# ewrfcas/MVSFormer

Hardware: AMD Instinct MI355X
Metric: depth maps/sec @1536x1152 N=5 D=192 (higher is better)
Workload: dtype f32

## Files before the change

### mvsformer_amd/csrc/vis_net_x3.hip

```cpp
#include <stdlib.h>

#include <type_traits>

#include "conv_common.h"
#include "split3.h"

#ifdef X3_ABLATE
#define VIS_ABLATE(a, bit) (((a) & (bit)) != 0)
static int vis_ablate_bits() { return mvs::env_int("MVS_VIS_ABLATE", 0); }
#else
#define VIS_ABLATE(a, bit) false
static constexpr int vis_ablate_bits() { return 0; }
#endif

namespace {
using namespace mvsconv;
using mvsx3::bf16x4;
using mvsx3::bf16x8;
using mvsx3::mfma6;
using mvsprim::u32x2;
using mvsx3::split3;

constexpr int T = 16;
constexpr int INW = T + 6, A1W = T + 4, A2W = T + 2;
constexpr int A1N = A1W * A1W, A2N = A2W * A2W;
constexpr int A1_OCT = A1N * 16, A1_TERM = 2 * A1_OCT;
constexpr int A2_OCT = A2N * 16, A2_TERM = 2 * A2_OCT;
constexpr int IN_BYTES = ((INW * INW * 4 + 255) / 256) * 256;
constexpr int IDX_BYTES = A1N * 4;
constexpr int LDS_BYTES = IN_BYTES + 3 * A1_TERM + 3 * A2_TERM + IDX_BYTES;
constexpr int L2_STEPS = 5, L3_STEPS = 6;
constexpr int L2_FLAT = A2W * A1W;
constexpr int L2_TILES = (L2_FLAT + 15) / 16, L1_TILES = A1N / 16;
static_assert(A1N % 16 == 0, "layer 1 tiles are full");
constexpr int OFF_W0 = 0, OFF_S0 = 144, OFF_B0 = 160, OFF_W1 = 176, OFF_S1 = 2480, OFF_B1 = 2496, OFF_W2 = 2512, OFF_S2 = 3664,
              OFF_B2 = 3672, OFF_W3 = 3680, OFF_B3 = 3688;

__global__ void vis_x3_prepare_kernel(const float* __restrict__ prm, bf16x8* __restrict__ out) {
    const int idx = blockIdx.x * blockDim.x + threadIdx.x;
    if (idx >= (L2_STEPS + L3_STEPS) * 3 * 64) return;
    const int lane = idx & 63, term = (idx >> 6) % 3, step = idx / 192;
    const int m = lane & 15, kb = lane >> 4;
    bf16x8 v;
#pragma unroll
    for (int e = 0; e < 8; ++e) {
        const int ci = (kb & 1) * 8 + e;
        float f = 0.0f;
        if (step < L2_STEPS) {
            const int tap = 2 * step + (kb >> 1);
            if (tap < 9) f = prm[OFF_W1 + (ci * 9 + tap) * 16 + m] * prm[OFF_S1 + m];
        } else {
            const int kblk = 2 * (step - L2_STEPS) + (kb >> 1), t = kblk / 3, kw = kblk % 3, dy = m >> 3, co = m & 7, kh = t - dy;
            if (kh >= 0 && kh <= 2) f = prm[OFF_W2 + (ci * 9 + kh * 3 + kw) * 8 + co] * prm[OFF_S2 + co];
        }
        __bf16 h, mm, l;
        split3(f, h, mm, l);
        v[e] = term == 0 ? h : (term == 1 ? mm : l);
    }
    out[idx] = v;
}

template <int OCT, int TERM>
__device__ __forceinline__ void store_split(unsigned char* base, int pix, int kb, const float (&v)[4]) {
    u32x2 h, m, l;
#pragma unroll
    for (int r = 0; r < 2; ++r) {
        unsigned a, b, c;
#ifdef VIS_SPLIT_CLAMPED
        mvsx3::split3_pair<true>(v[2 * r], v[2 * r + 1], a, b, c);
#else
        mvsx3::split3_pair<false>(v[2 * r], v[2 * r + 1], a, b, c);
#endif
        h[r] = a; m[r] = b; l[r] = c;
    }
    unsigned char* dst = base + (kb >> 1) * OCT + pix * 16 + (kb & 1) * 8;
    *reinterpret_cast<u32x2*>(dst) = h;
    *reinterpret_cast<u32x2*>(dst + TERM) = m;
    *reinterpret_cast<u32x2*>(dst + 2 * TERM) = l;
}

__global__ __launch_bounds__(256, 2) void vis_x3_kernel(const float* __restrict__ entropy, const float* __restrict__ prm,
                                                        const bf16x8* __restrict__ prep, int N, int H, int W, int ntx, int nty,
                                                        float* __restrict__ weight, int ablate) {
    extern __shared__ __attribute__((aligned(16))) unsigned char smem[];
    float* s_in = reinterpret_cast<float*>(smem);
    unsigned char* s_a1 = smem + IN_BYTES;
    unsigned char* s_a2 = s_a1 + 3 * A1_TERM;
    unsigned* s_idx = reinterpret_cast<unsigned*>(s_a2 + 3 * A2_TERM);
    const int tid = threadIdx.x, lane = tid & 63;
    const int wave = __builtin_amdgcn_readfirstlane(tid >> 6);
    const int n = lane & 15, kb = lane >> 4;

    bf16x8 w2[L2_STEPS][3], w3[L3_STEPS][3];
#pragma unroll
    for (int s = 0; s < L2_STEPS; ++s)
#pragma unroll
        for (int t = 0; t < 3; ++t) w2[s][t] = prep[(s * 3 + t) * 64 + lane];
#pragma unroll
    for (int s = 0; s < L3_STEPS; ++s)
#pragma unroll
        for (int t = 0; t < 3; ++t) w3[s][t] = prep[((L2_STEPS + s) * 3 + t) * 64 + lane];

    float W1A[3];
    int tap_off[3];
#pragma unroll
    for (int t = 0; t < 3; ++t) {
        const int tap = 4 * t + kb;
        W1A[t] = tap < 9 ? prm[OFF_W0 + tap * 16 + n] * prm[OFF_S0 + n] : 0.0f;
        const int tc = tap < 9 ? tap : 8;
        tap_off[t] = (tc / 3) * INW + tc % 3;
    }
    f32x4 sh0, sh1, sh2;
    float wl[4];
#pragma unroll
    for (int r = 0; r < 4; ++r) {
        sh0[r] = prm[OFF_B0 + 4 * kb + r];
        sh1[r] = prm[OFF_B1 + 4 * kb + r];
        const int co = (kb & 1) * 4 + r;
        sh2[r] = prm[OFF_B2 + co];
        wl[r] = prm[OFF_W3 + co];
    }
    const float b3 = prm[OFF_B3];
    unsigned off2[L2_STEPS], off3[L3_STEPS];
#pragma unroll
    for (int s = 0; s < L2_STEPS; ++s) {
        const int tap = min(2 * s + (kb >> 1), 8);
        off2[s] = (unsigned)((kb & 1) * A1_OCT + ((tap / 3) * A1W + tap % 3) * 16);
    }
#pragma unroll
    for (int s = 0; s < L3_STEPS; ++s) {
        const int kblk = 2 * s + (kb >> 1);
        off3[s] = (unsigned)((kb & 1) * A2_OCT + ((kblk / 3) * A2W + kblk % 3) * 16);
    }

    const int ntiles = N * ntx * nty;
    constexpr int EPT = (INW * INW + 255) / 256;
    float pre[EPT];
    auto tile_origin = [&](int tile, int& img, int& x0, int& y0) {
        img = tile / (ntx * nty);
        y0 = ((tile / ntx) % nty) * T;
        x0 = (tile % ntx) * T;
    };
    auto fetch_entropy = [&](int tile) {
        int img, x0, y0;
        tile_origin(tile, img, x0, y0);
        const float* src = entropy + (size_t)img * H * W;
#pragma unroll
        for (int e = 0; e < EPT; ++e) {
            const int i = tid + e * 256;
            const int gy = y0 - 3 + i / INW, gx = x0 - 3 + i % INW;
            pre[e] = (i < INW * INW && gy >= 0 && gy < H && gx >= 0 && gx < W) ? src[(size_t)gy * W + gx] : 0.0f;
        }
    };
    auto commit_entropy = [&]() {
#pragma unroll
        for (int e = 0; e < EPT; ++e)
            if (tid + e * 256 < INW * INW) s_in[tid + e * 256] = pre[e];
    };

    int tile = blockIdx.x;
    if (tile >= ntiles) return;
    fetch_entropy(tile);
    commit_entropy();
    for (int p = tid; p < A1N; p += 256) {
        const int py = p / A1W, px = p % A1W;
        s_idx[p] = (unsigned)((py * INW + px) * 4) | (unsigned)py << 16 | (unsigned)px << 24;
    }
    __syncthreads();
    for (; tile < ntiles; tile += gridDim.x) {
        int img, x0, y0;
        tile_origin(tile, img, x0, y0);
        const int next = tile + gridDim.x;
        const bool has_next = next < ntiles;
        if (has_next) fetch_entropy(next);

        const bool interior = x0 >= 2 && y0 >= 2 && x0 + T + 2 <= W && y0 + T + 2 <= H;

        auto layer1 = [&](auto inner) {
            constexpr bool INNER = decltype(inner)::value;
#pragma unroll 1
            for (int t = wave; t < L1_TILES && !VIS_ABLATE(ablate, 1); t += 4) {
                const int p = t * 16 + n;
                const unsigned ix = s_idx[p];
                const float* src = reinterpret_cast<const float*>(reinterpret_cast<const unsigned char*>(s_in) + (ix & 0xffffu));
                f32x4 z = sh0;
#pragma unroll
                for (int k = 0; k < 3; ++k) z = mfma4(W1A[k], src[tap_off[k]], z);
                float cap = __builtin_inff();
                if (!INNER) {
                    const int gy = y0 - 2 + (int)((ix >> 16) & 0xffu), gx = x0 - 2 + (int)(ix >> 24);
                    cap = (gy >= 0 && gy < H && gx >= 0 && gx < W) ? __builtin_inff() : 0.0f;
                }
                float v[4];
#pragma unroll
                for (int r = 0; r < 4; ++r) v[r] = INNER ? fmaxf(z[r], 0.0f) : __builtin_amdgcn_fmed3f(z[r], 0.0f, cap);
                store_split<A1_OCT, A1_TERM>(s_a1, p, kb, v);
            }
        };
        if (interior) layer1(std::true_type{}); else layer1(std::false_type{});
        __syncthreads();

#pragma unroll 1
        for (int t = wave; t < L2_TILES; t += 8) {
            const int o0 = t * 16 + n, o1 = min(t + 4, L2_TILES - 1) * 16 + n;
            const bool two = t + 4 < L2_TILES;
            const unsigned char* b0 = s_a1 + o0 * 16;
            const unsigned char* b1 = s_a1 + o1 * 16;
            f32x4 c0 = sh1, c1 = sh1;
            bf16x8 x0f[2][3], x1f[2][3];
#pragma unroll
            for (int k = 0; k < 3; ++k) {
                x0f[0][k] = *reinterpret_cast<const bf16x8*>(b0 + off2[0] + k * A1_TERM);
                x1f[0][k] = *reinterpret_cast<const bf16x8*>(b1 + off2[0] + k * A1_TERM);
            }
#ifndef VIS_SETPRIO
#define VIS_SETPRIO 1
#endif
            if (VIS_SETPRIO) __builtin_amdgcn_s_setprio(1);
#pragma unroll
            for (int s = 0; s < L2_STEPS; ++s) {
                if (s + 1 < L2_STEPS) {
#pragma unroll
                    for (int k = 0; k < 3; ++k) {
                        x0f[(s + 1) & 1][k] = *reinterpret_cast<const bf16x8*>(b0 + off2[s + 1] + k * A1_TERM);
                        x1f[(s + 1) & 1][k] = *reinterpret_cast<const bf16x8*>(b1 + off2[s + 1] + k * A1_TERM);
                    }
                }
                __builtin_amdgcn_sched_barrier(0);
                if (!VIS_ABLATE(ablate, 2)) {
                    c0 = mfma6(w2[s], x0f[s & 1], c0);
                    c1 = mfma6(w2[s], x1f[s & 1], c1);
                }
                __builtin_amdgcn_sched_barrier(0);
            }
            if (VIS_SETPRIO) __builtin_amdgcn_s_setprio(0);
            auto finish = [&](int tt, const f32x4& c) {
                const int o = tt * 16 + n, oy = o / A1W, ox = o % A1W;
                if (oy < A2W && ox < A2W) {
                    float v[4];
                    if (interior) {
#pragma unroll
                        for (int r = 0; r < 4; ++r) v[r] = fmaxf(c[r], 0.0f);
                    } else {
                        const int gy = y0 - 1 + oy, gx = x0 - 1 + ox;
                        const float cap = (gy >= 0 && gy < H && gx >= 0 && gx < W) ? __builtin_inff() : 0.0f;
#pragma unroll
                        for (int r = 0; r < 4; ++r) v[r] = __builtin_amdgcn_fmed3f(c[r], 0.0f, cap);
                    }
                    store_split<A2_OCT, A2_TERM>(s_a2, oy * A2W + ox, kb, v);
                }
            };
            if (!VIS_ABLATE(ablate, 4)) {
                finish(t, c0);
                if (two) finish(t + 4, c1);
            }
        }
        if (has_next) commit_entropy();
        __syncthreads();

        {
            const unsigned char* b0 = s_a2 + ((2 * wave) * A2W + n) * 16;
            const unsigned char* b1 = s_a2 + ((2 * (wave + 4)) * A2W + n) * 16;
            f32x4 c0 = sh2, c1 = sh2;
            bf16x8 x0f[2][3], x1f[2][3];
#pragma unroll
            for (int k = 0; k < 3; ++k) {
                x0f[0][k] = *reinterpret_cast<const bf16x8*>(b0 + off3[0] + k * A2_TERM);
                x1f[0][k] = *reinterpret_cast<const bf16x8*>(b1 + off3[0] + k * A2_TERM);
            }
            if (VIS_SETPRIO) __builtin_amdgcn_s_setprio(1);
#pragma unroll
            for (int s = 0; s < L3_STEPS; ++s) {
                if (s + 1 < L3_STEPS) {
#pragma unroll
                    for (int k = 0; k < 3; ++k) {
                        x0f[(s + 1) & 1][k] = *reinterpret_cast<const bf16x8*>(b0 + off3[s + 1] + k * A2_TERM);
                        x1f[(s + 1) & 1][k] = *reinterpret_cast<const bf16x8*>(b1 + off3[s + 1] + k * A2_TERM);
                    }
                }
                __builtin_amdgcn_sched_barrier(0);
                if (!VIS_ABLATE(ablate, 8)) {
                    c0 = mfma6(w3[s], x0f[s & 1], c0);
                    c1 = mfma6(w3[s], x1f[s & 1], c1);
                }
                __builtin_amdgcn_sched_barrier(0);
            }
            if (VIS_SETPRIO) __builtin_amdgcn_s_setprio(0);
            auto reduce = [&](const f32x4& c) {
                float part = 0.0f;
#pragma unroll
                for (int r = 0; r < 4; ++r) part = fmaf(wl[r], fmaxf(c[r], 0.0f), part);
                return part + __shfl_xor(part, 16, 64);
            };
            if (!VIS_ABLATE(ablate, 16)) {
                const float p0 = reduce(c0), p1 = reduce(c1);
                const bool second = (kb & 1) != 0;
                const float part = second ? p1 : p0;
                const int gy = y0 + 2 * (second ? wave + 4 : wave) + (kb >> 1), gx = x0 + n;
                if (gy < H && gx < W) weight[(size_t)img * H * W + (size_t)gy * W + gx] = 1.0f / (1.0f + expf(-(part + b3)));
            }
        }
    }
}

}

extern "C" int mvs_vis_x3_prepare(const float* params, void* prepared, mvs_stream_t stream) {
    MVS_REQUIRE(params && prepared, "mvs_vis_x3_prepare: null pointer");
    constexpr int total = (L2_STEPS + L3_STEPS) * 3 * 64;
    static_assert(total * 16 == MVS_VIS_X3_BYTES, "MVS_VIS_X3_BYTES");
    hipLaunchKernelGGL(vis_x3_prepare_kernel, dim3(mvs::ceil_div(total, 256)), dim3(256), 0, MVS_STREAM(stream), params, static_cast<bf16x8*>(prepared));
    return mvs::finish_launch("mvs_vis_x3_prepare");
}

extern "C" int mvs_vis_x3_fwd(const float* entropy, const float* params, const void* prepared, int N, int H, int W, float* weight,
                              mvs_stream_t stream) {
    MVS_REQUIRE(entropy && params && prepared && weight, "mvs_vis_x3_fwd: null pointer");
    MVS_REQUIRE(N >= 1 && H >= 1 && W >= 1, "mvs_vis_x3_fwd: bad shape N=%d H=%d W=%d", N, H, W);
    const int ntx = mvs::ceil_div(W, T), nty = mvs::ceil_div(H, T);
    MVS_REQUIRE((int64_t)N * ntx * nty < ((int64_t)1 << 31), "mvs_vis_x3_fwd: too many tiles");
    const int ncu = mvs::device_cus();
    const int ntiles = N * ntx * nty;
    const int blocks = ntiles < 2 * ncu ? ntiles : 2 * ncu;
    {
        const int rc = mvs::ensure_dynamic_lds(reinterpret_cast<const void*>(&vis_x3_kernel), LDS_BYTES, "mvs_vis_x3_fwd");
        if (rc != MVS_OK) return rc;
    }
    hipLaunchKernelGGL(vis_x3_kernel, dim3(blocks), dim3(256), LDS_BYTES, MVS_STREAM(stream), entropy, params, static_cast<const bf16x8*>(prepared), N,
                       H, W, ntx, nty, weight, vis_ablate_bits());
    return mvs::finish_launch("mvs_vis_x3_fwd");
}
```

Measured before the change: 269.1.

## Software-pipeline layer-2 epilogue into next tile's MFMA stream

Restructures the layer-2 conv loop so each wave processes one tile per pass and interleaves the previous tile's ReLU, bf16x3 split and LDS stores, one piece after each MFMA. A trash pixel slot is added to A2 so out-of-range outputs store unconditionally instead of branching. The goal is to hide epilogue VALU and LDS-store latency behind matrix instructions. In exchange the code is more complex, uses more registers, and loses the two-tile accumulator pairing, so MFMA dependency chains get longer.

```diff
diff --git a/mvsformer_amd/csrc/vis_net_x3.hip b/mvsformer_amd/csrc/vis_net_x3.hip
--- a/mvsformer_amd/csrc/vis_net_x3.hip
+++ b/mvsformer_amd/csrc/vis_net_x3.hip
@@ -1,6 +1,7 @@
 #include <stdlib.h>
 
 #include <type_traits>
+#include <utility>
 
 #include "conv_common.h"
 #include "split3.h"
@@ -25,7 +26,8 @@
 constexpr int INW = T + 6, A1W = T + 4, A2W = T + 2;
 constexpr int A1N = A1W * A1W, A2N = A2W * A2W;
 constexpr int A1_OCT = A1N * 16, A1_TERM = 2 * A1_OCT;
-constexpr int A2_OCT = A2N * 16, A2_TERM = 2 * A2_OCT;
+constexpr int A2_TRASH = A2N;
+constexpr int A2_OCT = (A2N + 1) * 16, A2_TERM = 2 * A2_OCT;
 constexpr int IN_BYTES = ((INW * INW * 4 + 255) / 256) * 256;
 constexpr int IDX_BYTES = A1N * 4;
 constexpr int LDS_BYTES = IN_BYTES + 3 * A1_TERM + 3 * A2_TERM + IDX_BYTES;
@@ -79,6 +81,67 @@
     *reinterpret_cast<u32x2*>(dst + 2 * TERM) = l;
 }
 
+struct L2Epi {
+    f32x4 c;
+    int o, oy, pix;
+    unsigned dst;
+    float cap;
+    f32x4 v;
+    mvsprim::f32x2 ra, rb;
+    u32x2 h, m, l;
+};
+constexpr int L2_EPI_STEPS = 22;
+static_assert(L2_EPI_STEPS <= 6 * L2_STEPS, "one piece behind each MFMA of a pass");
+template <int J, bool INNER>
+__device__ __forceinline__ void l2_epi_step(L2Epi& e, unsigned char* s_a2, unsigned st_lane, int x0, int y0, int H, int W) {
+    if constexpr (J == 0) {
+        e.oy = e.o / A1W;
+    } else if constexpr (J == 1) {
+        const int ox = e.o - e.oy * A1W;
+        e.pix = (e.oy < A2W && ox < A2W) ? e.oy * A2W + ox : A2_TRASH;
+        if (!INNER) {
+            const int gy = y0 - 1 + e.oy, gx = x0 - 1 + ox;
+            e.cap = (gy >= 0 && gy < H && gx >= 0 && gx < W) ? __builtin_inff() : 0.0f;
+        }
+    } else if constexpr (J == 2) {
+        e.dst = st_lane + (unsigned)e.pix * 16u;
+    } else if constexpr (J == 3 || J == 4) {
+#pragma unroll
+        for (int r = 2 * (J - 3); r < 2 * (J - 3) + 2; ++r) e.v[r] = INNER ? fmaxf(e.c[r], 0.0f) : __builtin_amdgcn_fmed3f(e.c[r], 0.0f, e.cap);
+    } else if constexpr (J >= 5 && J < 19) {
+        constexpr int r = (J - 5) & 1, P = (J - 5) >> 1;
+        if constexpr (P == 0) {
+#ifdef VIS_SPLIT_CLAMPED
+            e.h[r] = mvsx3::cvt_pk_bf16(__builtin_amdgcn_fmed3f(e.v[2 * r], -mvsx3::BF16_MAX, mvsx3::BF16_MAX),
+                                        __builtin_amdgcn_fmed3f(e.v[2 * r + 1], -mvsx3::BF16_MAX, mvsx3::BF16_MAX));
+#else
+            e.h[r] = mvsx3::cvt_pk_bf16(e.v[2 * r], e.v[2 * r + 1]);
+#endif
+        } else if constexpr (P == 1) {
+            e.ra[r] = e.v[2 * r] - __builtin_bit_cast(float, e.h[r] << 16);
+        } else if constexpr (P == 2) {
+            e.rb[r] = e.v[2 * r + 1] - __builtin_bit_cast(float, e.h[r] & 0xffff0000u);
+        } else if constexpr (P == 3) {
+            e.m[r] = mvsx3::cvt_pk_bf16(e.ra[r], e.rb[r]);
+        } else if constexpr (P == 4) {
+            e.ra[r] = e.ra[r] - __builtin_bit_cast(float, e.m[r] << 16);
+        } else if constexpr (P == 5) {
+            e.rb[r] = e.rb[r] - __builtin_bit_cast(float, e.m[r] & 0xffff0000u);
+        } else {
+            e.l[r] = mvsx3::cvt_pk_bf16(e.ra[r], e.rb[r]);
+        }
+    } else if constexpr (J == 19) {
+        *reinterpret_cast<u32x2*>(s_a2 + e.dst) = e.h;
+    } else if constexpr (J == 20) {
+        *reinterpret_cast<u32x2*>(s_a2 + e.dst + A2_TERM) = e.m;
+    } else if constexpr (J == 21) {
+        *reinterpret_cast<u32x2*>(s_a2 + e.dst + 2 * A2_TERM) = e.l;
+    }
+}
+template <class F, int... I>
+__device__ __forceinline__ void for_each_int(F&& f, std::integer_sequence<int, I...>) {
+    (f(std::integral_constant<int, I>{}), ...);
+}
 __global__ __launch_bounds__(256, 2) void vis_x3_kernel(const float* __restrict__ entropy, const float* __restrict__ prm,
                                                         const bf16x8* __restrict__ prep, int N, int H, int W, int ntx, int nty,
                                                         float* __restrict__ weight, int ablate) {
@@ -132,6 +195,7 @@
         const int kblk = 2 * s + (kb >> 1);
         off3[s] = (unsigned)((kb & 1) * A2_OCT + ((kblk / 3) * A2W + kblk % 3) * 16);
     }
+    const unsigned st_lane = (unsigned)((kb >> 1) * A2_OCT + (kb & 1) * 8);
 
     const int ntiles = N * ntx * nty;
     constexpr int EPT = (INW * INW + 255) / 256;
@@ -200,61 +264,53 @@
         if (interior) layer1(std::true_type{}); else layer1(std::false_type{});
         __syncthreads();
 
-#pragma unroll 1
-        for (int t = wave; t < L2_TILES; t += 8) {
-            const int o0 = t * 16 + n, o1 = min(t + 4, L2_TILES - 1) * 16 + n;
-            const bool two = t + 4 < L2_TILES;
-            const unsigned char* b0 = s_a1 + o0 * 16;
-            const unsigned char* b1 = s_a1 + o1 * 16;
-            f32x4 c0 = sh1, c1 = sh1;
-            bf16x8 x0f[2][3], x1f[2][3];
-#pragma unroll
-            for (int k = 0; k < 3; ++k) {
-                x0f[0][k] = *reinterpret_cast<const bf16x8*>(b0 + off2[0] + k * A1_TERM);
-                x1f[0][k] = *reinterpret_cast<const bf16x8*>(b1 + off2[0] + k * A1_TERM);
-            }
 #ifndef VIS_SETPRIO
 #define VIS_SETPRIO 1
 #endif
+        auto layer2 = [&](auto inner) {
+            constexpr bool INNER = decltype(inner)::value;
+            auto frag = [&](bf16x8 (&x)[3], int t, int s) {
+                const unsigned char* b = s_a1 + (t * 16 + n) * 16 + off2[s];
+#pragma unroll
+                for (int k = 0; k < 3; ++k) x[k] = *reinterpret_cast<const bf16x8*>(b + k * A1_TERM);
+            };
+            auto pass = [&](int t, auto defer, L2Epi& e, bf16x8 (&xs)[3][3]) {
+                constexpr bool DEFER = decltype(defer)::value;
+                constexpr int WI[6] = {1, 2, 0, 1, 0, 0}, XI[6] = {1, 0, 2, 0, 1, 0};
+                f32x4 c = sh1;
+                auto slot = [&](auto ic) {
+                    constexpr int I = decltype(ic)::value, s = I / 6, j = I % 6;
+                    bf16x8 (&x)[3] = xs[s == 0 ? 0 : 1 + ((s - 1) & 1)];
+                    if (!VIS_ABLATE(ablate, 2)) c = __builtin_amdgcn_mfma_f32_16x16x32_bf16(w2[s][WI[j]], x[XI[j]], c, 0, 0, 0);
+                    if (j == 0) {
+                        if (s + 1 < L2_STEPS) frag(xs[1 + (s & 1)], t, s + 1);
+                        else frag(xs[0], min(t + 4, L2_TILES - 1), 0);
+                    }
+                    if (DEFER && !VIS_ABLATE(ablate, 4)) l2_epi_step<I, INNER>(e, s_a2, st_lane, x0, y0, H, W);
+                    __builtin_amdgcn_sched_barrier(0);
+                };
+                for_each_int(slot, std::make_integer_sequence<int, 6 * L2_STEPS>{});
+                return c;
+            };
+            bf16x8 xs[3][3];
+            L2Epi e;
+            int t = wave;
+            frag(xs[0], t, 0);
             if (VIS_SETPRIO) __builtin_amdgcn_s_setprio(1);
-#pragma unroll
-            for (int s = 0; s < L2_STEPS; ++s) {
-                if (s + 1 < L2_STEPS) {
-#pragma unroll
-                    for (int k = 0; k < 3; ++k) {
-                        x0f[(s + 1) & 1][k] = *reinterpret_cast<const bf16x8*>(b0 + off2[s + 1] + k * A1_TERM);
-                        x1f[(s + 1) & 1][k] = *reinterpret_cast<const bf16x8*>(b1 + off2[s + 1] + k * A1_TERM);
-                    }
-                }
-                __builtin_amdgcn_sched_barrier(0);
-                if (!VIS_ABLATE(ablate, 2)) {
-                    c0 = mfma6(w2[s], x0f[s & 1], c0);
-                    c1 = mfma6(w2[s], x1f[s & 1], c1);
-                }
-                __builtin_amdgcn_sched_barrier(0);
+            e.c = pass(t, std::false_type{}, e, xs);
+#pragma unroll 1
+            for (t += 4; t < L2_TILES; t += 4) {
+                e.o = (t - 4) * 16 + n;
+                const f32x4 c = pass(t, std::true_type{}, e, xs);
+                e.c = c;
             }
             if (VIS_SETPRIO) __builtin_amdgcn_s_setprio(0);
-            auto finish = [&](int tt, const f32x4& c) {
-                const int o = tt * 16 + n, oy = o / A1W, ox = o % A1W;
-                if (oy < A2W && ox < A2W) {
-                    float v[4];
-                    if (interior) {
-#pragma unroll
-                        for (int r = 0; r < 4; ++r) v[r] = fmaxf(c[r], 0.0f);
-                    } else {
-                        const int gy = y0 - 1 + oy, gx = x0 - 1 + ox;
-                        const float cap = (gy >= 0 && gy < H && gx >= 0 && gx < W) ? __builtin_inff() : 0.0f;
-#pragma unroll
-                        for (int r = 0; r < 4; ++r) v[r] = __builtin_amdgcn_fmed3f(c[r], 0.0f, cap);
-                    }
-                    store_split<A2_OCT, A2_TERM>(s_a2, oy * A2W + ox, kb, v);
-                }
-            };
-            if (!VIS_ABLATE(ablate, 4)) {
-                finish(t, c0);
-                if (two) finish(t + 4, c1);
-            }
-        }
+            e.o = (t - 4) * 16 + n;
+            if (!VIS_ABLATE(ablate, 4))
+                for_each_int([&](auto j) { l2_epi_step<decltype(j)::value, INNER>(e, s_a2, st_lane, x0, y0, H, W); },
+                             std::make_integer_sequence<int, L2_EPI_STEPS>{});
+        };
+        if (interior) layer2(std::true_type{}); else layer2(std::false_type{});
         if (has_next) commit_entropy();
         __syncthreads();
 
```

Result: no change. 271.1 (median of 6 runs) (+0.7%).
